# mcomunita/syncfusion

Measured on AMD Instinct MI355X. Metric: U-Net denoise steps/sec (batch x 2 s@22.05 kHz), higher is better.
Workload: dtype bf16; 1 GPU; BASELINE configs[1]: batch=8/GPU, 50-step DDIM (v-sampler) denoising of 2 s @ 22.05 kHz clips (L0=45056 = 44*1024, cropped to 44100), bf16, embedding_scale=1.0 (1 U-Net eval/step), dummy cond; this run timed 1568 consecutive sampler steps (the cost of a step does not depend on the schedule length); batch_per_gpu=8, L0=45056, hip_graph=True, weights_broadcast_bytes=0, gathered_clips=8

## Files before the change

include/syncfusion_amd.h:

```cpp
#ifndef SYNCFUSION_AMD_H
#define SYNCFUSION_AMD_H

#include <stdint.h>

#ifdef __cplusplus
extern "C" {
#endif

#define SF_MAX_DEPTH 12

enum {
  SF_OK = 0,
  SF_ERR_INVALID = 1,
  SF_ERR_MISSING_WEIGHT = 2,
  SF_ERR_SHAPE = 3,
  SF_ERR_HIP = 4,
  SF_ERR_WORKSPACE = 5,
  SF_ERR_UNSUPPORTED = 6
};

enum { SF_UP_NEAREST_CONV3 = 0, SF_UP_TRANSPOSE = 1 };
enum { SF_F32 = 0, SF_BF16 = 1, SF_F16 = 2, SF_F32X = 3 };

typedef struct {
// ... 129 lines not shown
                        int B, int L, int C, int N, int taps, int pad, float *dx, float *dw, float *db, float *dgb, void *ws,
                        int64_t ws_bytes, void *stream);
int64_t sf_op_gn_silu_train_stats_floats(int B, int L, int C, int groups);
int sf_op_gn_silu_train(const float *x, const float *gamma, const float *beta, int groups, float eps, int B, int L, int C, float *act, float *stats,
                        void *stream);
int sf_op_conv1d_bwd_cl_act(const float *x, const float *act, const float *stats , const float *w, const float *gamma, const float *beta,
                            int groups, float eps, const float *dy, int B, int L, int C, int N, int taps, int pad, float *dx, float *dw, float *db,
                            float *dgb, void *ws, int64_t ws_bytes, void *stream);
int sf_op_conv1d_bwd_cl_x(int dtype, const float *x, const float *act, const float *stats, const float *w, const float *gamma, const float *beta,
                          int groups, float eps, const float *dy, int B, int L, int C, int N, int taps, int pad, float *dx, float *dw, float *db,
                          float *dgb, void *ws, int64_t ws_bytes, void *stream);
int64_t sf_op_conv1d_dgrad_pack_bytes(int C, int N, int taps);
int sf_op_conv1d_train_fwd(int dtype, const float *x, const float *w, const float *bias, const float *gamma, const float *beta, int groups, float eps,
                           const float *residual, int B, int L, int C, int N, int taps, int pad, float *out, void *dgrad_pack, int64_t dgrad_pack_bytes,
                           void *ws, int64_t ws_bytes, void *stream);
int sf_op_conv1d_bwd_cl_p(int dtype, const float *x, const float *act, const float *stats, const float *w, const void *dgrad_pack, const float *gamma,
                          const float *beta, int groups, float eps, const float *dy, const float *dx_add, int B, int L, int C, int N, int taps, int pad,
                          float *dx, float *dw, float *db, float *dgb, void *ws, int64_t ws_bytes, void *stream);
int sf_op_conv1d_train_images(int dtype, const float *w, int B, int L, int C, int N, int taps, int pad, int groups);
int sf_op_conv1d_variant(int dtype, int B, int L, int C, int N, int taps, int stride, int pad, int upsample, int groups, char *label, int label_bytes);
int sf_op_conv1d_bwd_variant(int dtype, int B, int L, int C, int N, int taps, int pad, char *label, int label_bytes);
int sf_train_pack_many(const void *desc_dev, int n_items, int total_tiles, void *stream);
int sf_op_conv1d_train_fwd_pk(int dtype, const float *x, const float *w, const float *fw, const void *fwx, const float *bias, const float *gamma,
                              const float *beta, int groups, float eps, const float *residual, int B, int L, int C, int N, int taps, int pad, float *out,
                              void *ws, int64_t ws_bytes, void *stream);
int sf_op_ln_modulate_bwd_add(const float *x, const float *scale_shift, const float *dy, const float *dx_add, float eps, int B, int L, int C, float *dx,
                              float *dss, void *ws, int64_t ws_bytes, void *stream);
int64_t sf_op_length_sums_workspace_bytes(int B, int L, int C);
int sf_op_length_sums(const float *x, const float *y , int B, int L, int C, float *out , void *ws, int64_t ws_bytes,
                      void *stream);
int64_t sf_op_ln_modulate_bwd_workspace_bytes(int B, int L, int C);
int sf_op_ln_modulate_bwd(const float *x, const float *scale_shift, const float *dy, float eps, int B, int L, int C, float *dx, float *dss,
                          void *ws, int64_t ws_bytes, void *stream);
int sf_op_attention_bwd(const float *q, const float *kv, const float *out, const float *dout, int B, int L, int heads, int head_dim, float *dq,
                        float *dkv, void *ws, int64_t ws_bytes, void *stream);
int sf_op_attention_fwd_lse(const float *q, const float *kv, int B, int L, int heads, int head_dim, float *out, float *lse, void *stream);
int sf_op_attention_fwd_lse_x(int dtype, const float *q, const float *kv, int B, int L, int heads, int head_dim, float *out, float *lse, void *stream);
int sf_op_attention_bwd_lse(const float *q, const float *kv, const float *out, const float *dout, const float *lse, int B, int L, int heads, int head_dim,
                            float *dq, float *dkv, void *ws, int64_t ws_bytes, void *stream);
int sf_op_attention_bwd_lse_x(int dtype, const float *q, const float *kv, const float *out, const float *dout, const float *lse, int B, int L, int heads,
                              int head_dim, float *dq, float *dkv, void *ws, int64_t ws_bytes, void *stream);
int sf_bench_conv1d(int dtype, int B, int L, int C, int N, int taps, int upsample, int path, int tile, int sk, int iters,
                    float *ms_out);
int64_t sf_op_resnet_mod_cb_workspace_bytes(int B, int L, int C);
int sf_op_resnet_mod_cb(int dtype, const void *x, const float *w1, const float *b1, const float *w2, const float *b2, const float *gn1_g,
                        const float *gn1_b, const float *gn2_g, const float *gn2_b, int groups, float eps_gn, const float *scale_shift,
                        float eps_ln, int B, int L, int C, int kb , void *h_out, void *m_out,
                        void *ws, int64_t ws_bytes, void *stream);
int64_t sf_op_resnet_mod_cbd_workspace_bytes(int B, int L, int C, int C2);
int sf_op_resnet_mod_cbd(int dtype, const void *x, const float *w1, const float *b1, const float *w2, const float *b2, const float *gn1_g,
                         const float *gn1_b, const float *gn2_g, const float *gn2_b, int groups, float eps_gn, const float *scale_shift,
                         float eps_ln, int B, int L, int C, const float *w_inj, const float *b_inj, const void *ctx, int ctx_ld, int C2,
                         const float *badd, void *h_out, void *m_out, void *z_out, float *stats_out, void *ws, int64_t ws_bytes, void *stream);
int64_t sf_op_inject_prenorm_proj_workspace_bytes(int B, int L, int C, int C2, int N);
int sf_op_inject_prenorm_proj(int dtype, const void *m, const void *ctx, const float *w_inj, const float *b_inj, const float *gamma,
                              const float *beta, float eps, const float *w_q, int B, int L, int C, int C2, int N, void *z_out, void *q_out,
                              int *fused_out, void *ws, int64_t ws_bytes, void *stream);
int sf_bench_conv_cb(int dtype, int B, int L, int C, int groups, int kb, int cold, int iters, float *ms );
int sf_op_gn_silu(int dtype, const void *x, const float *gamma, const float *beta, int groups, float eps, int B, int L, int C, void *out,
                  void *ws, int64_t ws_bytes, void *stream);
int sf_op_ln_modulate(int dtype, const void *x, const float *scale_shift , float eps,
                      int B, int L, int C, void *out, void *stream);
int sf_op_attention(int dtype, const void *q, const void *kv, int B, int L, int heads, int head_dim, void *out, void *stream);


typedef struct {
  int32_t N, T, Hi, Wi;
  int32_t cin, cin_ld;
  int32_t cout, cout_ld;
  int32_t kt, kh, kw;
  int32_t sh, sw;
  int32_t pt, ph, pw;
} sf_vconv_desc;
int64_t sf_op_vconv_workspace_bytes(const sf_vconv_desc *desc );
int sf_op_vconv_fwd(const sf_vconv_desc *desc, const float *x, const float *w, float *y, void *ws, int64_t ws_bytes, void *stream);
int sf_op_vconv_bwd(const sf_vconv_desc *desc, const float *x, const float *w, const float *dy, float *dx, float *dw, void *ws, int64_t ws_bytes,
                    void *stream);
int64_t sf_op_bn_train_workspace_bytes(int64_t rows, int C);
int sf_op_bn_train_fwd(const float *x, const float *res, int64_t rows, int C, int ld, const float *gamma, const float *beta, float eps, float momentum,
                       float *running_mean, float *running_var, int64_t *num_batches_tracked, int relu, float *y, float *save_mean, float *save_invstd,
                       void *ws, int64_t ws_bytes, void *stream);
int sf_op_bn_train_bwd(const float *x, const float *y, const float *dy, int64_t rows, int C, int ld, const float *gamma, const float *save_mean,
                       const float *save_invstd, float *dx, float *dres, float *dgamma, float *dbeta, void *ws, int64_t ws_bytes, void *stream);
int64_t sf_op_bn_sync_workspace_bytes(int64_t rows, int C);
int sf_op_bn_sync_stats(const float *x, int64_t rows, int C, int ld, float *local_stats, void *ws, int64_t ws_bytes, void *stream);
int sf_op_bn_sync_fwd_apply(const float *x, const float *res, int64_t rows, int C, int ld, const float *gathered_stats, const int64_t *row_counts, int world,
                            const float *gamma, const float *beta, float eps, float momentum, float *running_mean, float *running_var,
                            int64_t *num_batches_tracked, int relu, float *y, float *save_mean, float *save_invstd, void *ws, int64_t ws_bytes,
                            void *stream);
int sf_op_bn_sync_bwd_sums(const float *x, const float *y, const float *dy, int64_t rows, int C, int ld, const float *save_mean, const float *save_invstd,
                           float *local_sums, float *dgamma, float *dbeta, void *ws, int64_t ws_bytes, void *stream);
int sf_op_bn_sync_bwd_apply(const float *x, const float *y, const float *dy, int64_t rows, int C, int ld, const float *gathered_sums,
                            const int64_t *row_counts, int world, const float *gamma, const float *save_mean, const float *save_invstd, float *dx,
                            float *dres, void *ws, int64_t ws_bytes, void *stream);
int sf_op_video_to_cl(const float *x, int N, int C, int T, int H, int W, int ld, float *out, void *stream);
int sf_op_video_pool(const float *x, int64_t NT, int HW, int C, int ld, float *out, void *stream);
int sf_op_video_pool_bwd(const float *dout, int64_t NT, int HW, int C, int ld, float *dx, void *stream);

int64_t sf_op_onset_loss_workspace_bytes(int64_t n);
int sf_op_onset_bce_fwd(const float *z, const float *t, int64_t n, float *loss, float *stats, void *ws, int64_t ws_bytes, void *stream);
int sf_op_onset_bce_bwd(const float *z, const float *t, const float *stats, const float *g, int64_t n, float *dz, void *stream);
int sf_op_onset_metrics(const float *z, const float *t, int N, int T, float threshold, double *out, void *ws, int64_t ws_bytes, void *stream);

int64_t sf_op_onset_test_workspace_bytes(int N, int T);
int sf_op_onset_test_step(const float *logits, const float *labels, int N, int T, float logit_threshold, float metric_threshold, int64_t clip0,
                          int64_t capacity, int32_t *pred_count, int32_t *pred_frames, int32_t *target_count, int32_t *target_frames,
// ... 41 lines not shown
```

syncfusion_amd/_lib.py:

```python
from __future__ import annotations

import ctypes as C
import os
from typing import Dict, Iterable, List, Optional, Sequence, Tuple

import torch

SF_MAX_DEPTH = 12
SF_F32, SF_BF16, SF_F16, SF_F32X = 0, 1, 2, 3
UPSAMPLE_MODES = {"nearest": 0, "transpose": 1}
DTYPES = {"fp32": SF_F32, "float32": SF_F32, "f32": SF_F32, "bf16": SF_BF16, "bfloat16": SF_BF16, "fp16": SF_F16, "float16": SF_F16, "f16": SF_F16, "half": SF_F16,
          "fp32x": SF_F32X}

_HERE = os.path.dirname(os.path.abspath(__file__))
LIB_PATH = os.environ.get("SF_LIB_PATH") or os.path.join(_HERE, "lib", "libsyncfusion_amd.so")


class SfTensor(C.Structure):
    _fields_ = [("name", C.c_char_p), ("data", C.c_void_p), ("numel", C.c_int64)]


class UnetConfig(C.Structure):
    _fields_ = [
        ("n_layers", C.c_int32), ("in_channels", C.c_int32),
# ... 52 lines not shown
    "sf_onsetnet_create": (_I, [C.POINTER(SfTensor), _I, _I, _P, C.POINTER(_P)]),
    "sf_onsetnet_destroy": (None, [_P]),
    "sf_onsetnet_workspace_bytes": (_L, [_P, _I, _I, _I, _I]),
    "sf_onsetnet_forward": (_I, [_P, _P, _I, _I, _I, _I, _P, _P, _L, _P]),
    "sf_onsetnet_debug_enable": (_I, [_P, _P, _L]),
    "sf_onsetnet_debug_count": (_I, [_P]),
    "sf_onsetnet_debug_detail": (_I, [_P, _I, C.POINTER(C.c_int32), _I]),
    "sf_onsetnet_debug_path": (_I, [_P, _I]),
    "sf_onsetnet_debug_info": (_I, [_P, _I, C.c_char_p, _I, C.POINTER(_L), C.POINTER(_L), C.POINTER(C.c_int32)]),
    "sf_onsets_to_track": (_I, [_P, _I, _I, _P, _F, _F, _F, _P, _I, _P]),
    "sf_frames_preprocess": (_I, [_P, _I, _I, _I, _I, _I, _I, _P, _P, _P, _P]),
    "sf_frames_augment_workspace_bytes": (_L, [_I, _I, _I, _I]),
    "sf_frames_augment": (_I, [_P, _I, _I, _I, _I, _I, _I, _I, _I, _P, _P, _P, _P, _P, _P, _L, _P]),
    "sf_times_to_track": (_I, [_P, _P, _I, C.c_double, _I, _I, _P, _P]),
    "sf_cut_prefix_crop": (_I, [_P, _P, _I, _I, _I, _I, _P, _P, _P]),
    "sf_resampler_create": (_I, [_I, _I, _I, _F, C.POINTER(_P)]),
    "sf_resampler_destroy": (None, [_P]),
    "sf_resampler_out_length": (_I, [_P, _I]),
    "sf_resampler_forward": (_I, [_P, _P, _I, _I, _P, _P]),
    "sf_op_conv1d_cl": (_I, [_I, _P, _P, _P, _P, _P, _I, _F, _P, _I, _I, _I, _I, _I, _I, _I, _I, _P, _P, _L, _P]),
    "sf_op_conv1d_bwd_workspace_bytes": (_L, [_I, _I, _I, _I, _I, _I]),
    "sf_op_conv1d_bwd_cl": (_I, [_P, _P, _P, _P, _I, _F, _P, _I, _I, _I, _I, _I, _I, _P, _P, _P, _P, _P, _L, _P]),
    "sf_op_conv1d_bwd_cl_act": (_I, [_P, _P, _P, _P, _P, _P, _I, _F, _P, _I, _I, _I, _I, _I, _I, _P, _P, _P, _P, _P, _L, _P]),
    "sf_op_conv1d_bwd_cl_x": (_I, [_I, _P, _P, _P, _P, _P, _P, _I, _F, _P, _I, _I, _I, _I, _I, _I, _P, _P, _P, _P, _P, _L, _P]),
    "sf_op_conv1d_dgrad_pack_bytes": (_L, [_I, _I, _I]),
    "sf_op_conv1d_train_fwd": (_I, [_I, _P, _P, _P, _P, _P, _I, _F, _P, _I, _I, _I, _I, _I, _I, _P, _P, _L, _P, _L, _P]),
    "sf_op_conv1d_bwd_cl_p": (_I, [_I, _P, _P, _P, _P, _P, _P, _P, _I, _F, _P, _P, _I, _I, _I, _I, _I, _I, _P, _P, _P, _P, _P, _L, _P]),
    "sf_op_conv1d_train_images": (_I, [_I, _P, _I, _I, _I, _I, _I, _I, _I]),
    "sf_op_conv1d_variant": (_I, [_I, _I, _I, _I, _I, _I, _I, _I, _I, _I, C.c_char_p, _I]),
    "sf_op_conv1d_bwd_variant": (_I, [_I, _I, _I, _I, _I, _I, _I, C.c_char_p, _I]),
    "sf_train_pack_many": (_I, [_P, _I, _I, _P]),
    "sf_op_conv1d_train_fwd_pk": (_I, [_I, _P, _P, _P, _P, _P, _P, _P, _I, _F, _P, _I, _I, _I, _I, _I, _I, _P, _P, _L, _P]),
    "sf_op_ln_modulate_bwd_add": (_I, [_P, _P, _P, _P, _F, _I, _I, _I, _P, _P, _P, _L, _P]),
    "sf_op_gn_silu_train_stats_floats": (_L, [_I, _I, _I, _I]),
    "sf_op_gn_silu_train": (_I, [_P, _P, _P, _I, _F, _I, _I, _I, _P, _P, _P]),
    "sf_op_ln_modulate_bwd_workspace_bytes": (_L, [_I, _I, _I]),
    "sf_op_ln_modulate_bwd": (_I, [_P, _P, _P, _F, _I, _I, _I, _P, _P, _P, _L, _P]),
    "sf_op_attention_bwd": (_I, [_P, _P, _P, _P, _I, _I, _I, _I, _P, _P, _P, _L, _P]),
    "sf_op_attention_fwd_lse": (_I, [_P, _P, _I, _I, _I, _I, _P, _P, _P]),
    "sf_op_attention_fwd_lse_x": (_I, [_I, _P, _P, _I, _I, _I, _I, _P, _P, _P]),
    "sf_op_attention_bwd_lse": (_I, [_P, _P, _P, _P, _P, _I, _I, _I, _I, _P, _P, _P, _L, _P]),
    "sf_op_attention_bwd_lse_x": (_I, [_I, _P, _P, _P, _P, _P, _I, _I, _I, _I, _P, _P, _P, _L, _P]),
    "sf_op_length_sums_workspace_bytes": (_L, [_I, _I, _I]),
    "sf_op_length_sums": (_I, [_P, _P, _I, _I, _I, _P, _P, _L, _P]),
    "sf_bench_conv1d": (_I, [_I, _I, _I, _I, _I, _I, _I, _I, _I, _I, _I, C.POINTER(C.c_float)]),
    "sf_op_gn_silu": (_I, [_I, _P, _P, _P, _I, _F, _I, _I, _I, _P, _P, _L, _P]),
    "sf_op_inject_prenorm_proj_workspace_bytes": (_L, [_I, _I, _I, _I, _I]),
    "sf_op_inject_prenorm_proj": (_I, [_I, _P, _P, _P, _P, _P, _P, _F, _P, _I, _I, _I, _I, _I, _P, _P, _P, _P, _L, _P]),
    "sf_op_resnet_mod_cb_workspace_bytes": (_L, [_I, _I, _I]),
    "sf_op_resnet_mod_cb": (_I, [_I, _P, _P, _P, _P, _P, _P, _P, _P, _P, _I, _F, _P, _F, _I, _I, _I, _I, _P, _P, _P, _L, _P]),
    "sf_op_resnet_mod_cbd_workspace_bytes": (_L, [_I, _I, _I, _I]),
    "sf_op_resnet_mod_cbd": (_I, [_I, _P, _P, _P, _P, _P, _P, _P, _P, _P, _I, _F, _P, _F, _I, _I, _I, _P, _P, _P, _I, _I, _P, _P, _P, _P, _P, _P,
                                  _L, _P]),
    "sf_bench_conv_cb": (_I, [_I, _I, _I, _I, _I, _I, _I, _I, C.POINTER(C.c_float)]),
    "sf_op_ln_modulate": (_I, [_I, _P, _P, _F, _I, _I, _I, _P, _P]),
    "sf_op_attention": (_I, [_I, _P, _P, _I, _I, _I, _I, _P, _P]),
    "sf_op_vconv_workspace_bytes": (_L, [C.POINTER(VConvDesc)]),
    "sf_op_vconv_fwd": (_I, [C.POINTER(VConvDesc), _P, _P, _P, _P, _L, _P]),
    "sf_op_vconv_bwd": (_I, [C.POINTER(VConvDesc), _P, _P, _P, _P, _P, _P, _L, _P]),
    "sf_op_bn_train_workspace_bytes": (_L, [_L, _I]),
    "sf_op_bn_train_fwd": (_I, [_P, _P, _L, _I, _I, _P, _P, _F, _F, _P, _P, _P, _I, _P, _P, _P, _P, _L, _P]),
    "sf_op_bn_train_bwd": (_I, [_P, _P, _P, _L, _I, _I, _P, _P, _P, _P, _P, _P, _P, _P, _L, _P]),
    "sf_op_bn_sync_workspace_bytes": (_L, [_L, _I]),
    "sf_op_bn_sync_stats": (_I, [_P, _L, _I, _I, _P, _P, _L, _P]),
    "sf_op_bn_sync_fwd_apply": (_I, [_P, _P, _L, _I, _I, _P, _P, _I, _P, _P, _F, _F, _P, _P, _P, _I, _P, _P, _P, _P, _L, _P]),
    "sf_op_bn_sync_bwd_sums": (_I, [_P, _P, _P, _L, _I, _I, _P, _P, _P, _P, _P, _P, _L, _P]),
    "sf_op_bn_sync_bwd_apply": (_I, [_P, _P, _P, _L, _I, _I, _P, _P, _I, _P, _P, _P, _P, _P, _P, _L, _P]),
    "sf_op_video_to_cl": (_I, [_P, _I, _I, _I, _I, _I, _I, _P, _P]),
    "sf_op_video_pool": (_I, [_P, _L, _I, _I, _I, _P, _P]),
    "sf_op_video_pool_bwd": (_I, [_P, _L, _I, _I, _I, _P, _P]),
    "sf_op_onset_loss_workspace_bytes": (_L, [_L]),
    "sf_op_onset_bce_fwd": (_I, [_P, _P, _L, _P, _P, _P, _L, _P]),
    "sf_op_onset_bce_bwd": (_I, [_P, _P, _P, _P, _L, _P, _P]),
    "sf_op_onset_metrics": (_I, [_P, _P, _I, _I, _F, _P, _P, _L, _P]),
    "sf_op_onset_test_workspace_bytes": (_L, [_I, _I]),
    "sf_op_onset_test_step": (_I, [_P, _P, _I, _I, _F, _F, _L, _L, _P, _P, _P, _P, _P, _P, _L, _P]),
    "sf_optim_workspace_bytes": (_L, [_I]),
    "sf_optim_adamw_step": (_I, [_P, _I, _I, _P, _I, _I, _P, _P, _L, _P]),
    "sf_audio_features_create": (_I, [_I, _I, _I, _I, _P, _P, _P, _L, C.POINTER(_P)]),
    "sf_audio_features_destroy": (None, [_P]),
    "sf_audio_features_workspace_bytes": (_L, [_P, _I, _I]),
    "sf_logmel_forward": (_I, [_P, _P, _I, _I, _F, _F, _P, _P, _P, _L, _P]),
    "sf_onset_detect": (_I, [_P, _P, _I, _I, _F, _F, _I, _I, _I, _I, _I, _I, _F, _I, _I, _P, _P, _P, _P, _P, _P, _L, _P]),
    "sf_audio_features_create_framed": (_I, [_I, _I, _I, _I, _P, _P, _P, _L, C.POINTER(_P)]),
    "sf_logmel_examples_count": (_I, [_P, _I, _I]),
    "sf_logmel_examples_forward": (_I, [_P, _P, _I, _I, _I, _F, _P, _P, _P]),
    "sf_vggish_create": (_I, [_I, _P, _I, _P, _I, _I, _I, _P, _P, _P, _P, _P, C.POINTER(_P)]),
    "sf_vggish_destroy": (None, [_P]),
    "sf_vggish_max_examples": (_I, [_P]),
    "sf_vggish_workspace_bytes": (_L, [_P, _I]),
    "sf_vggish_forward": (_I, [_P, _P, _I, _P, _P, _P, _L, _P]),
    "sf_op_maxpool2x2_cl": (_I, [_P, _L, _I, _I, _I, _P, _P]),
    "sf_op_moments": (_I, [_P, _L, _I, _P, _P, _P]),
}

_lib: Optional[C.CDLL] = None


class SyncFusionAmdError(RuntimeError):
    pass


def load() -> C.CDLL:
    global _lib
    if _lib is not None:
        return _lib
# ... 56 lines not shown
```

syncfusion_amd/csrc/capi_misc.cpp:

```cpp
#include <algorithm>
#include <cstring>
#include <cstdlib>
#include <cmath>
#include <exception>

#include "engine_common.h"

using namespace sf;

#define SF_API_BEGIN try {
#define SF_API_END                  \
  }                                 \
  catch (const EngineError &e) {    \
    return e.code;                  \
  }                                 \
  catch (const std::exception &e) { \
    set_error("%s", e.what());      \
    return SF_ERR_INVALID;          \
  }

extern "C" {

const char *sf_version(void) { return "syncfusion_amd 0.1.0 (gfx950)"; }
const char *sf_last_error(void) { return get_error(); }
// ... 580 lines not shown
  Workspace wk(ws, ws_bytes);
  const int64_t es = 2;
  char *wp = static_cast<char *>(wk.alloc(2 * (int64_t)C * C * 3 * es));
  void *wp1 = wp, *wp2 = wp + (int64_t)C * C * 3 * es;
  void *act = wk.alloc(M * C * es);
  void *h = h_out ? h_out : wk.alloc(M * C * es);
  void *m = m_out ? m_out : wk.alloc(M * C * es);
  float *stats = stats_out ? stats_out : static_cast<float *>(wk.alloc((int64_t)B * 32 * 64 * 2 * 4));
  if (w_inj) {
    void *wi = wk.alloc((int64_t)C * (C + C2) * es);
    ai.w = wi;
    ai.src = ai.res = m;
    if (!conv_gemm_supported(dtype, ai)) fail(SF_ERR_UNSUPPORTED, "InjectChannels shape outside the GEMM kernels' coverage");
    SF_HIP(launch_pack_rows(dtype, w_inj, C, C + C2, C + C2, nullptr, wi, C + C2, s));
  }
  SF_HIP(launch_pack_conv_cb(dtype, w1, C, C, wp1, s));
  SF_HIP(launch_pack_conv_cb(dtype, w2, C, C, wp2, s));
  SF_HIP(launch_gn_silu(dtype, x, C, B, L, C, groups, gn1_g, gn1_b, eps_gn, act, C, s));
  ConvCbArgs a;
  a.src = act;
  a.src_ld = C;
  a.wp = wp1;
  a.B = B;
  a.L = L;
  a.C = a.N = C;
  a.G = groups;
  const CbGnPlan gp = cb_gn_plan(L);
  a.nch = gp.nch;
  a.chunk_rows = gp.chunk_rows;
  a.epi = 1;
  a.out = h;
  a.out_ld = C;
  a.bias = b1;
  a.stats_out = stats;
  SF_HIP(launch_conv_cb(dtype, a, s));
  a.src = h;
  a.wp = wp2;
  a.pro = 1;
  a.stats = stats;
  a.gamma = gn2_g;
  a.beta = gn2_b;
  a.eps = eps_gn;
  a.epi = 2;
  a.out = m;
  a.bias = b2;
  a.stats_out = nullptr;
  a.res = x;
  a.res_ld = C;
  a.ss = scale_shift;
  a.ss_ld = 2 * C;
  a.eps_ln = eps_ln;
  SF_HIP(launch_conv_cb(dtype, a, s));
  if (w_inj) SF_HIP(launch_conv_gemm(dtype, ai, s));
  return SF_OK;
  SF_API_END
}

int64_t sf_op_inject_prenorm_proj_workspace_bytes(int B, int L, int C, int C2, int N) {
  if (B < 1 || L < 1 || C < 32 || C2 < 0 || N < 8) return -1;
  const int64_t M = (int64_t)B * L, K1 = C + (C2 + 31) / 32 * 32;
  return (int64_t)C * K1 * 2 + (int64_t)N * C * 2 + M * C * 2 + M * (C / 32) * 8 + (int64_t)(2 * N + C) * 4 + 4096;
}

int sf_op_inject_prenorm_proj(int dtype, const void *m, const void *ctx, const float *w_inj, const float *b_inj, const float *gamma,
                              const float *beta, float eps, const float *w_q, int B, int L, int C, int C2, int N, void *z_out, void *q_out,
                              int *fused_out, void *ws, int64_t ws_bytes, void *stream) {
  SF_API_BEGIN
  if (!m || !w_inj || !b_inj || !gamma || !beta || !w_q || !z_out || !q_out || !ws) fail(SF_ERR_INVALID, "null argument");
  if (dtype != BF16 && dtype != F16) fail(SF_ERR_UNSUPPORTED, "16-bit dtypes only");
  if (C % 32 || C2 % 32 || N % 32 || (C2 > 0 && !ctx)) fail(SF_ERR_UNSUPPORTED, "C, C2 and N must be multiples of 32");
  const int64_t need = sf_op_inject_prenorm_proj_workspace_bytes(B, L, C, C2, N);
  if (need < 0 || ws_bytes < need) fail(SF_ERR_WORKSPACE, "workspace too small: need %lld bytes", (long long)need);
  hipStream_t s = static_cast<hipStream_t>(stream);
  Workspace wk(ws, ws_bytes);
  const int64_t M = (int64_t)B * L;
  const int K1 = C + C2;
  void *w1 = wk.alloc((int64_t)C * K1 * 2), *w2 = wk.alloc((int64_t)N * C * 2), *tmp = wk.alloc(M * C * 2);
  float *rowpart = static_cast<float *>(wk.alloc(M * (C / 32) * 8));
  float *bias2 = static_cast<float *>(wk.alloc((int64_t)N * 4)), *colsum = static_cast<float *>(wk.alloc((int64_t)N * 4));
  SF_HIP(launch_pack_rows(dtype, w_inj, C, K1, K1, nullptr, w1, K1, s));
  SF_HIP(launch_pack_rows(dtype, w_q, N, C, C, gamma, w2, C, s));
  SF_HIP(launch_fold_bias(w_q, N, C, beta, nullptr, bias2, s));
  SF_HIP(launch_row_sums(dtype, w2, N, C, colsum, s));
  ConvGemmArgs a;
  a.src = m;
  a.src_ld = C;
  a.src2 = ctx;
  a.src2_ld = C2;
  a.w = w1;
  a.bias = b_inj;
  a.M = (int)M;
  a.N = a.n_store = C;
  a.K = K1;
  a.cin = C;
  a.cin2 = C2;
  a.taps = 1;
  a.Lout = a.Lsrc = L;
  a.out = z_out;
  a.out_ld = C;
  a.res = m;
  a.res_ld = C;
  ConvGemmArgs q;
  q.src = z_out;
  q.src_ld = C;
  q.w = w2;
  q.bias = bias2;
// ... 119 lines not shown
```

syncfusion_amd/csrc/conv_thin.hip:

```cpp
#include <cstdlib>
#include <type_traits>

#include "common.h"
#include "kernels.h"

namespace sf {
namespace {

static int thin_max_waves(int C) {
  static const int v32 = [] {
    const char *e = tune_env("SF_THIN_WAVES32");
    const int w = e ? atoi(e) : 8;
    return w >= 16 ? 16 : (w >= 8 ? 8 : 4);
  }();
  static const int v64 = [] {
    const char *e = tune_env("SF_THIN_WAVES64");
    const int w = e ? atoi(e) : 8;
    return w >= 16 ? 16 : (w >= 8 ? 8 : 4);
  }();
  return C == 32 ? v32 : (C == 64 ? v64 : 16);
}

constexpr int kThinMaxTiles = 64;
constexpr int kThinMaxG = 16;
// ... 86 lines not shown
  __device__ __forceinline__ static K8x zero() {
    K8x r;
    const u32x4 z = {0u, 0u, 0u, 0u};
    r.h = __builtin_bit_cast(f16x8, z);
    r.l = r.h;
    return r;
  }
};
__device__ __forceinline__ void mma_step_x3(f32x16 &accM, f32x16 &accL, const K8x &a, const K8x &b) { x3_mfma<X3_F16>(a.h, a.l, b.h, b.l, accM, accL); }
__device__ __forceinline__ void x3_fold(f32x16 &accM, const f32x16 &accL) {
#pragma unroll
  for (int i = 0; i < 16; ++i) accM[i] = fmaf(accL[i], X3P<X3_F16>::INV, accM[i]);
}

template <int CTRL, int ROW_MASK> __device__ __forceinline__ float dpp_mov(float v) {
  return __int_as_float(__builtin_amdgcn_update_dpp(0, __float_as_int(v), CTRL, ROW_MASK, 0xf, false));
}
__device__ __forceinline__ float2 half_sums(float v) {
  v += dpp_mov<0xb1, 0xf>(v);
  v += dpp_mov<0x4e, 0xf>(v);
  v += dpp_mov<0x124, 0xf>(v);
  v += dpp_mov<0x128, 0xf>(v);
  v += dpp_mov<0x142, 0xa>(v);
  return make_float2(__int_as_float(__builtin_amdgcn_readlane(__float_as_int(v), 31)),
                     __int_as_float(__builtin_amdgcn_readlane(__float_as_int(v), 63)));
}
__device__ __forceinline__ float half_sum32(float v, int half) {
  v += dpp_mov<0xb1, 0xf>(v);
  v += dpp_mov<0x4e, 0xf>(v);
  v += dpp_mov<0x124, 0xf>(v);
  v += dpp_mov<0x128, 0xf>(v);
  v += dpp_mov<0x142, 0xa>(v);
  const float lo = __int_as_float(__builtin_amdgcn_readlane(__float_as_int(v), 31));
  const float hi = __int_as_float(__builtin_amdgcn_readlane(__float_as_int(v), 63));
  return half ? hi : lo;
}

template <bool FAST = false>
__device__ __forceinline__ float2 gn_merge_n(const float *__restrict__ sl, int G, int nch, int chunk_rows, int L, int cpg, float eps,
                                             int lane32) {
  float n = 0.f, mean = 0.f, m2 = 0.f;
  for (int i = lane32; i < nch; i += 32) {
    const int rows = min(chunk_rows, L - i * chunk_rows);
    welford_merge_t<FAST>(n, mean, m2, (float)rows * (float)cpg, sl[(size_t)i * G * 2], sl[(size_t)i * G * 2 + 1]);
  }
#pragma unroll
  for (int off = 16; off > 0; off >>= 1) {
    const float nb = __shfl_down(n, off, 32), mb = __shfl_down(mean, off, 32), qb = __shfl_down(m2, off, 32);
    welford_merge_t<FAST>(n, mean, m2, nb, mb, qb);
  }
  const float mu = __shfl(mean, 0, 32), var = div_t<FAST>(__shfl(m2, 0, 32), __shfl(n, 0, 32));
  return make_float2(mu, rsqrtf(var + eps));
}

template <typename T> struct K4;
template <> struct K4<bf16> {
  uint2 raw;
  __device__ __forceinline__ float get(int i) const {
    const unsigned int w = i < 2 ? raw.x : raw.y;
    return __uint_as_float((i & 1) ? (w & 0xffff0000u) : (w << 16));
  }
  __device__ __forceinline__ static K4 load(const bf16 *p) {
    K4 r;
    r.raw = *reinterpret_cast<const uint2 *>(p);
    return r;
  }
  __device__ __forceinline__ static K4 zero() {
    K4 r;
    r.raw = make_uint2(0u, 0u);
    return r;
  }
};
template <> struct K4<f16> {
  typedef __attribute__((ext_vector_type(4))) _Float16 f16x4;
  f16x4 v;
  __device__ __forceinline__ float get(int i) const { return (float)v[i]; }
  __device__ __forceinline__ static K4 load(const f16 *p) {
    K4 r;
    r.v = *reinterpret_cast<const f16x4 *>(p);
    return r;
  }
  __device__ __forceinline__ static K4 zero() {
    K4 r;
    r.v = f16x4{(f16)0.f, (f16)0.f, (f16)0.f, (f16)0.f};
    return r;
  }
};
template <> struct K4<float> {
  f32x4 v;
  __device__ __forceinline__ float get(int i) const { return v[i]; }
  __device__ __forceinline__ static K4 load(const float *p) {
    K4 r;
    r.v = *reinterpret_cast<const f32x4 *>(p);
    return r;
  }
  __device__ __forceinline__ static K4 zero() {
    K4 r;
    r.v = f32x4{0.f, 0.f, 0.f, 0.f};
    return r;
  }
};

template <typename T, int CIN, int TAPS, int C2, int PRO, int NOUT, bool X3 = false>
__global__ __launch_bounds__(X3 ? 512 : 1024) void conv_thin_kernel(const ConvThinArgs a) {
  static_assert(!X3 || sizeof(T) == 4, "split mode: fp32 activations");
  constexpr int E = 8;
// ... 344 lines not shown
  nw = (nw / NCB) * NCB;
  if (((a.rw >> a.up_shift) + 3) * (CIN / 8) > 6 * nw * 64) return hipErrorInvalidValue;
  hipLaunchKernelGGL(kern, dim3(a.B * a.nchw), dim3(nw * 64), lds, s, a);
  return hipGetLastError();
}

struct ThinShape {
  int cin, taps, c2, pro, nout;
};
constexpr ThinShape kThinShapes[] = {
    {8, 3, 0, 1, 8},   {32, 3, 0, 1, 32},  {64, 3, 0, 1, 64},
    {8, 1, 8, 2, 8},   {32, 1, 32, 2, 32}, {64, 1, 32, 2, 64}, {64, 1, 64, 2, 64},
    {32, 1, 0, 0, 32}, {64, 1, 0, 0, 64},  {128, 1, 0, 0, 64},
    {32, 3, 0, 0, 8},  {64, 3, 0, 0, 32},  {64, 3, 0, 0, 64},
};

static hipError_t thin_dispatch_x3(const ConvThinArgs &a, hipStream_t s) {
#define SF_THINX(CC, TT, C22, PP, NN) \
  if (a.C == CC && a.taps == TT && a.C2 == C22 && a.pro == PP && a.N == NN) return thin_go<float, CC, TT, C22, PP, NN, true>(a, s)
  SF_THINX(32, 3, 0, 1, 32);
  SF_THINX(64, 3, 0, 1, 64);
  SF_THINX(32, 1, 32, 2, 32);
  SF_THINX(64, 1, 32, 2, 64);
  SF_THINX(64, 1, 64, 2, 64);
  SF_THINX(32, 1, 0, 0, 32);
  SF_THINX(64, 1, 0, 0, 64);
  SF_THINX(128, 1, 0, 0, 64);
  SF_THINX(64, 3, 0, 0, 32);
  SF_THINX(64, 3, 0, 0, 64);
#undef SF_THINX
  return hipErrorInvalidValue;
}

template <typename T> hipError_t thin_dispatch(const ConvThinArgs &a, hipStream_t s) {
#define SF_THIN(CC, TT, C22, PP, NN) \
  if (a.C == CC && a.taps == TT && a.C2 == C22 && a.pro == PP && a.N == NN) return thin_go<T, CC, TT, C22, PP, NN>(a, s)
  SF_THIN(8, 3, 0, 1, 8);
  SF_THIN(32, 3, 0, 1, 32);
  SF_THIN(64, 3, 0, 1, 64);
  SF_THIN(8, 1, 8, 2, 8);
  SF_THIN(32, 1, 32, 2, 32);
  SF_THIN(64, 1, 32, 2, 64);
  SF_THIN(64, 1, 64, 2, 64);
  SF_THIN(32, 1, 0, 0, 32);
  SF_THIN(64, 1, 0, 0, 64);
  SF_THIN(128, 1, 0, 0, 64);
  SF_THIN(32, 3, 0, 0, 8);
  SF_THIN(64, 3, 0, 0, 32);
  SF_THIN(64, 3, 0, 0, 64);
#undef SF_THIN
  return hipErrorInvalidValue;
}

template <typename T, int C, int C2, bool X3 = false>
__global__ __launch_bounds__(X3 ? 512 : 1024) void thin_tail_kernel(const ThinTailArgs a) {
  static_assert(!X3 || sizeof(T) == 4, "split mode: fp32 activations");
  constexpr int E = 8;
  constexpr int QC = C / E;
  constexpr int S2 = 3 * QC, NST2 = (S2 + 1) / 2;
  constexpr int NSTM = (C + 15) / 16;
  constexpr int SC = C2 / E, NSTC = (SC + 1) / 2;
  constexpr int NCB = (C + 31) / 32;
  constexpr int K2 = 3 * C, K3 = C + C2;
  constexpr int P2 = K2 + E, P3 = K3 + E;
  constexpr int SROW = C + E;
  constexpr int NV = 6;
  constexpr bool FAST = !std::is_same<T, float>::value;

  extern __shared__ __align__(16) unsigned char smem[];
  float *sc = reinterpret_cast<float *>(smem);
  float *sh = sc + C;
  float *lsc = sh + C;
  float *lsh = lsc + C;
  float *ep = lsh + C;
  float *part = ep + 128;
  T *w2s = reinterpret_cast<T *>(part + kThinMaxTiles * kThinMaxG * 2);
  T *w3s = w2s + C * P2;
  T *tile = w3s + C * P3;
  f16 *w2H = reinterpret_cast<f16 *>(w2s), *w2L = w2H + C * P2;
  f16 *w3H = reinterpret_cast<f16 *>(w3s), *w3L = w3H + C * P3;
  f16 *tileH = reinterpret_cast<f16 *>(tile), *tileL = tileH + (size_t)(a.rw + 4) * SROW;

  const int tid = threadIdx.x, lane = tid & 63, wave = tid >> 6, NW = blockDim.x >> 6;
  const int half = lane >> 5, l32 = lane & 31;
  const int b = blockIdx.x / a.nchw, ch = blockIdx.x - b * a.nchw;
  const int r0 = ch * a.rw;
  const int rows = min(a.rw, a.L - r0);
  const int ntile = (rows + 31) >> 5;
  const int cpg = C / a.G;
  const T *src = static_cast<const T *>(a.h);

  const int total = (rows + 2) * QC;
  K8<T> xin[NV];
#pragma unroll
  for (int i = 0; i < NV; ++i) {
    const int idx = tid + i * blockDim.x;
    const int rr = idx / QC, q = idx - rr * QC;
    const int pos = r0 - 1 + rr;
    const bool ok = idx < total && pos >= 0 && pos < a.L;
    xin[i] = ok ? K8<T>::load(src + ((size_t)b * a.L + pos) * C + q * E) : K8<T>::zero();
  }
  for (int i = tid; i < C * (K2 / E); i += blockDim.x) {
    const int r = i / (K2 / E), v = i - r * (K2 / E);
    const K8<T> w = K8<T>::load(static_cast<const T *>(a.w2) + (size_t)r * K2 + v * E);
    if constexpr (X3) K8x::from(w).store(w2H + r * P2 + v * E, w2L + r * P2 + v * E);
    else w.store(w2s + r * P2 + v * E);
  }
  for (int i = tid; i < C * (K3 / E); i += blockDim.x) {
    const int r = i / (K3 / E), v = i - r * (K3 / E);
    const K8<T> w = K8<T>::load(static_cast<const T *>(a.w3) + (size_t)r * K3 + v * E);
    if constexpr (X3) K8x::from(w).store(w3H + r * P3 + v * E, w3L + r * P3 + v * E);
    else w.store(w3s + r * P3 + v * E);
  }
  for (int g = tid >> 5; g < a.G; g += blockDim.x >> 5) {
    const float2 st = gn_merge_n<FAST>(a.stats_in + ((size_t)b * a.nch_in * a.G + g) * 2, a.G, a.nch_in, a.chunk_in, a.L, cpg, a.eps_gn, l32);
    if (l32 < cpg) {
      const int c = g * cpg + l32;
      const float s = st.y * a.gamma[c];
      sc[c] = s;
      sh[c] = a.beta[c] - st.x * s;
    }
  }
  if (tid < C) {
    lsc[tid] = 1.0f + a.ss[(size_t)b * a.ss_ld + tid];
    lsh[tid] = a.ss[(size_t)b * a.ss_ld + C + tid];
    ep[tid] = a.bias2[tid];
    ep[64 + tid] = a.bias3[tid] + (a.badd ? a.badd[(size_t)b * a.badd_ld + tid] : 0.f);
  }
  __syncthreads();
#pragma unroll
  for (int i = 0; i < NV; ++i) {
    const int idx = tid + i * blockDim.x;
    if (idx < total) {
      const int rr = idx / QC, q = idx - rr * QC;
      const int pos = r0 - 1 + rr;
      const bool ok = pos >= 0 && pos < a.L;
      K8<T> v = xin[i];
#pragma unroll
      for (int e = 0; e < E; ++e) {
        const float y = fmaf(v.get(e), sc[q * E + e], sh[q * E + e]);
        v.set(e, ok ? silu_t<FAST>(y) : 0.f);
      }
      if constexpr (X3) K8x::from(v).store(tileH + rr * SROW + q * E, tileL + rr * SROW + q * E);
      else v.store(tile + rr * SROW + q * E);
    }
  }
  __syncthreads();

  for (int t = wave; t < ntile; t += NW) {
    const int row_l = t * 32 + l32;
    const bool rvalid = row_l < rows;
    const size_t grow = (size_t)b * a.L + r0 + (rvalid ? row_l : 0);
    K8<T> cf[NSTC > 0 ? NSTC : 1];
#pragma unroll
    for (int i = 0; i < NSTC; ++i) {
      const int q2 = 2 * i + half;
      cf[i] = (rvalid && q2 < SC) ? K8<T>::load(static_cast<const T *>(a.ctx) + grow * a.ctx_ld + q2 * E) : K8<T>::zero();
    }
    K4<T> rxf[NCB][4];
#pragma unroll
    for (int cb = 0; cb < NCB; ++cb)
#pragma unroll
      for (int v = 0; v < 4; ++v) {
        const int c0 = cb * 32 + half * 4 + 8 * v;
        rxf[cb][v] = (c0 < C && rvalid) ? K4<T>::load(static_cast<const T *>(a.x) + grow * C + c0) : K4<T>::zero();
      }
    f32x16 acc[NCB];
#pragma unroll
    for (int cb = 0; cb < NCB; ++cb)
#pragma unroll
      for (int i = 0; i < 16; ++i) acc[cb][i] = 0.f;
    const int prow = rvalid ? row_l : 0;
    if constexpr (X3) {
      f32x16 accL[NCB];
#pragma unroll
      for (int cb = 0; cb < NCB; ++cb)
#pragma unroll
        for (int i = 0; i < 16; ++i) accL[cb][i] = 0.f;
#pragma unroll
      for (int s = 0; s < NST2; ++s) {
// ... 196 lines not shown
            pp[1] = q;
          }
        }
      } else {
        const float cnt = (float)vrows * (float)cpg;
#pragma unroll
        for (int cb = 0; cb < NCB; ++cb)
#pragma unroll
          for (int v = 0; v < 4; ++v) {
            const float2 hs = half_sums((xs[cb][v][0] + xs[cb][v][1]) + (xs[cb][v][2] + xs[cb][v][3]));
            const float m = div_t<FAST>(cpg == 8 ? hs.x + hs.y : (half ? hs.y : hs.x), cnt);
            float q = 0.f;
#pragma unroll
            for (int e = 0; e < 4; ++e) {
              const float d = rvalid ? xs[cb][v][e] - m : 0.f;
              q = fmaf(d, d, q);
            }
            const float2 hq = half_sums(q);
            const float qq = cpg == 8 ? hq.x + hq.y : (half ? hq.y : hq.x);
            if (l32 == 0 && (cpg == 4 || half == 0)) {
              float *pp = part + ((size_t)t * a.G + (cb * 32 + half * 4 + 8 * v) / cpg) * 2;
              pp[0] = m;
              pp[1] = qq;
            }
          }
      }
    }
  }
  if (a.stats_out) {
    __syncthreads();
    for (int g = wave; g < a.G; g += NW) {
      const bool on = lane < ntile;
      const float *pp = part + ((size_t)(on ? lane : 0) * a.G + g) * 2;
      const float n_t = on ? (float)min(32, rows - lane * 32) * (float)cpg : 0.f;
      const float m_t = on ? pp[0] : 0.f, q_t = on ? pp[1] : 0.f;
      const float2 sn = half_sums(n_t), sm = half_sums(n_t * m_t);
      const float n = sn.x + sn.y, mean = div_t<FAST>(sm.x + sm.y, n);
      const float d = m_t - mean;
      const float2 sq2 = half_sums(fmaf(n_t * d, d, q_t));
      if (lane == 0) {
        float *so = a.stats_out + (((size_t)b * a.nchw + ch) * a.G + g) * 2;
        so[0] = mean;
        so[1] = sq2.x + sq2.y;
      }
    }
  }
}

template <typename T> size_t tail_lds_bytes(int C, int C2, int rw) {
  return (size_t)(4 * C + 128 + kThinMaxTiles * kThinMaxG * 2) * sizeof(float) +
         ((size_t)C * (3 * C + 8) + (size_t)C * (C + C2 + 8) + (size_t)(rw + 4) * (C + 8)) * sizeof(T);
}

template <typename T, int C, int C2, bool X3 = false> hipError_t tail_go(const ThinTailArgs &a, hipStream_t s) {
  const size_t lds = tail_lds_bytes<T>(C, C2, a.rw);
  auto kern = thin_tail_kernel<T, C, C2, X3>;
  if (lds > 64 * 1024) {
    static bool raised = false;
    if (!raised) {
      hipError_t e = hipFuncSetAttribute(reinterpret_cast<const void *>(kern), hipFuncAttributeMaxDynamicSharedMemorySize, 160 * 1024);
      if (e != hipSuccess) return e;
      raised = true;
    }
  }
  int nw = (a.rw + 31) / 32;
  if (nw > thin_max_waves(C)) nw = thin_max_waves(C);
  if (X3 && nw > 8) nw = 8;
  if ((a.rw + 2) * (C / 8) > 6 * nw * 64) return hipErrorInvalidValue;
  hipLaunchKernelGGL(kern, dim3(a.B * a.nchw), dim3(nw * 64), lds, s, a);
  return hipGetLastError();
}

template <typename T> hipError_t tail_dispatch(const ThinTailArgs &a, hipStream_t s) {
  if (a.C == 8 && a.C2 == 8) return tail_go<T, 8, 8>(a, s);
  if (a.C == 32 && a.C2 == 32) return tail_go<T, 32, 32>(a, s);
  if (a.C == 64 && a.C2 == 32) return tail_go<T, 64, 32>(a, s);
  if (a.C == 64 && a.C2 == 64) return tail_go<T, 64, 64>(a, s);
  return hipErrorInvalidValue;
}

}

bool thin_tail_supported(int dt, const ThinTailArgs &a) {
  const bool shape = (a.C == 8 && a.C2 == 8) || (a.C == 32 && a.C2 == 32) || (a.C == 64 && (a.C2 == 32 || a.C2 == 64));
  if (!shape || a.rw < 32 || a.rw % 32 || a.rw > 32 * kThinMaxTiles) return false;
  if (a.G < 1 || a.G > kThinMaxG || a.C % a.G) return false;
  const int cpg = a.C / a.G;
  if (a.C == 8 ? cpg != 1 : (cpg != 4 && cpg != 8)) return false;
  if (!a.ss || !a.stats_in) return false;
  {
    int nw = (a.rw + 31) / 32;
    if (nw > thin_max_waves(a.C)) nw = thin_max_waves(a.C);
    if ((a.rw + 2) * (a.C / 8) > 6 * nw * 64) return false;
  }
  const size_t lds = dt == F32 ? tail_lds_bytes<float>(a.C, a.C2, a.rw) : tail_lds_bytes<bf16>(a.C, a.C2, a.rw);
  return lds <= 160 * 1024;
}

hipError_t launch_thin_tail(int dt, const ThinTailArgs &a, hipStream_t s) {
  if (!thin_tail_supported(dt, a)) return hipErrorInvalidValue;
  if (d0_tail_supported(a)) return launch_d0_tail(dt, a, s);
  if (dt == F32 && a.x3) {
    if (a.C == 32 && a.C2 == 32) return tail_go<float, 32, 32, true>(a, s);
    if (a.C == 64 && a.C2 == 32) return tail_go<float, 64, 32, true>(a, s);
    if (a.C == 64 && a.C2 == 64) return tail_go<float, 64, 64, true>(a, s);
  }
  return SF_DISPATCH_T(dt, tail_dispatch<T>(a, s));
}

ThinPlan conv_thin_plan(int B, int L, int C) {
  ThinPlan p;
  static const int rows8 = [] {
    const char *e = tune_env("SF_THIN_ROWS8");
    const int v = e ? atoi(e) : 0;
    return v > 0 ? v : 0;
  }();
  static const int rows_cap = [] {
    const char *e = tune_env("SF_THIN_MAXROWS");
    const int v = e ? atoi(e) : 0;
    return v > 0 ? v : 352;
  }();
  static const int rows32 = [] {
    const char *e = tune_env("SF_THIN_MAXROWS32");
    const int v = e ? atoi(e) : 0;
    return v > 0 ? v : 512;
  }();
  const int max_rows = C <= 8 ? (rows8 > 0 ? rows8 : (d0_enabled(B, L) ? 992 : 2048)) : (C == 32 && rows32 > 0 ? rows32 : rows_cap);
  static const int wgs = [] {
    const char *e = tune_env("SF_THIN_WGS");
    const int v = e ? atoi(e) : 0;
    return v > 0 ? v : 256;
  }();
  long target = ((long)B * L + wgs - 1) / wgs;
  int rw = (int)((target + 31) / 32) * 32;
  if (rw < 32) rw = 32;
  if (rw > max_rows) rw = max_rows;
  p.rw = rw;
  p.nchw = (L + rw - 1) / rw;
  return p;
}

bool conv_thin_supported(int dt, const ConvThinArgs &a) {
  bool shape = false;
  for (const ThinShape &t : kThinShapes) shape = shape || (a.C == t.cin && a.taps == t.taps && a.C2 == t.c2 && a.pro == t.pro && a.N == t.nout);
  if (!shape) return false;
// ... 31 lines not shown
```

Baseline: 540.4 steps/s.

## Stage thin-tail weights and GroupNorm stats up front with overlapped loads

Adds an AHEAD variant of the thin-level tail kernel for 16-bit dtypes with C>=32 and small row windows. It issues the weight loads into registers in batches, and folds the GroupNorm statistics (with an FMA/reciprocal Welford merge) while those loads are in flight. The goal is to hide global-load latency during the prologue. It also enforces a minimum wave count, tunable by env, for these small blocks, and exposes a standalone C API entry point for the tail. The cost is more register pressure and a lower launch bound of 512.

Result: faster. 549.9 steps/s (median of 6 runs) (+1.8%).

```diff
diff --git a/include/syncfusion_amd.h b/include/syncfusion_amd.h
--- a/include/syncfusion_amd.h
+++ b/include/syncfusion_amd.h
@@ -205,6 +205,11 @@
                          const float *gn1_b, const float *gn2_g, const float *gn2_b, int groups, float eps_gn, const float *scale_shift,
                          float eps_ln, int B, int L, int C, const float *w_inj, const float *b_inj, const void *ctx, int ctx_ld, int C2,
                          const float *badd, void *h_out, void *m_out, void *z_out, float *stats_out, void *ws, int64_t ws_bytes, void *stream);
+int64_t sf_op_thin_tail_workspace_bytes(int dtype, int C, int C2);
+int sf_op_thin_tail(int dtype, const void *h, const void *x, const void *ctx, int ctx_ld, int c2_real, int C2, const float *stats_in, int nch_in,
+                    int chunk_in, const float *w2, const float *b2, const float *gn_g, const float *gn_b, int groups, float eps_gn,
+                    const float *scale_shift, float eps_ln, const float *w_inj, const float *b_inj, const float *badd, int B, int L, int C, int rw,
+                    void *z_out, float *stats_out, int *rw_out, void *ws, int64_t ws_bytes, void *stream);
 int64_t sf_op_inject_prenorm_proj_workspace_bytes(int B, int L, int C, int C2, int N);
 int sf_op_inject_prenorm_proj(int dtype, const void *m, const void *ctx, const float *w_inj, const float *b_inj, const float *gamma,
                               const float *beta, float eps, const float *w_q, int B, int L, int C, int C2, int N, void *z_out, void *q_out,
diff --git a/syncfusion_amd/_lib.py b/syncfusion_amd/_lib.py
--- a/syncfusion_amd/_lib.py
+++ b/syncfusion_amd/_lib.py
@@ -128,6 +128,9 @@
     "sf_op_resnet_mod_cbd_workspace_bytes": (_L, [_I, _I, _I, _I]),
     "sf_op_resnet_mod_cbd": (_I, [_I, _P, _P, _P, _P, _P, _P, _P, _P, _P, _I, _F, _P, _F, _I, _I, _I, _P, _P, _P, _I, _I, _P, _P, _P, _P, _P, _P,
                                   _L, _P]),
+    "sf_op_thin_tail_workspace_bytes": (_L, [_I, _I, _I]),
+    "sf_op_thin_tail": (_I, [_I, _P, _P, _P, _I, _I, _I, _P, _I, _I, _P, _P, _P, _P, _I, _F, _P, _F, _P, _P, _P, _I, _I, _I, _I, _P, _P,
+                             C.POINTER(C.c_int), _P, _L, _P]),
     "sf_bench_conv_cb": (_I, [_I, _I, _I, _I, _I, _I, _I, _I, C.POINTER(C.c_float)]),
     "sf_op_ln_modulate": (_I, [_I, _P, _P, _F, _I, _I, _I, _P, _P]),
     "sf_op_attention": (_I, [_I, _P, _P, _I, _I, _I, _I, _P, _P]),
diff --git a/syncfusion_amd/csrc/capi_misc.cpp b/syncfusion_amd/csrc/capi_misc.cpp
--- a/syncfusion_amd/csrc/capi_misc.cpp
+++ b/syncfusion_amd/csrc/capi_misc.cpp
@@ -656,6 +656,72 @@
   a.eps_ln = eps_ln;
   SF_HIP(launch_conv_cb(dtype, a, s));
   if (w_inj) SF_HIP(launch_conv_gemm(dtype, ai, s));
+  return SF_OK;
+  SF_API_END
+}
+
+int64_t sf_op_thin_tail_workspace_bytes(int dtype, int C, int C2) {
+  if ((dtype != F32 && dtype != BF16 && dtype != F16) || C < 1 || C2 < 0) return -1;
+  Workspace dry(nullptr, 0);
+  dry.alloc((int64_t)C * 3 * C * (int64_t)dsize(dtype));
+  dry.alloc((int64_t)C * (C + C2) * (int64_t)dsize(dtype));
+  return dry.used();
+}
+
+int sf_op_thin_tail(int dtype, const void *h, const void *x, const void *ctx, int ctx_ld, int c2_real, int C2, const float *stats_in, int nch_in,
+                    int chunk_in, const float *w2, const float *b2, const float *gn_g, const float *gn_b, int groups, float eps_gn,
+                    const float *scale_shift, float eps_ln, const float *w_inj, const float *b_inj, const float *badd, int B, int L, int C, int rw,
+                    void *z_out, float *stats_out, int *rw_out, void *ws, int64_t ws_bytes, void *stream) {
+  SF_API_BEGIN
+  if (!h || !x || !stats_in || !w2 || !b2 || !gn_g || !gn_b || !scale_shift || !w_inj || !b_inj || !z_out || !ws) fail(SF_ERR_INVALID, "null argument");
+  if (dtype != F32 && dtype != BF16 && dtype != F16) fail(SF_ERR_UNSUPPORTED, "dtype: fp32, bf16 or fp16");
+  if (B < 1 || L < 1 || C < 8) fail(SF_ERR_INVALID, "bad shape");
+  if (C2 < 0 || C2 % 8 || c2_real < 0 || c2_real > C2 || (C2 > 0 && (!ctx || ctx_ld < C2 || ctx_ld % 8))) fail(SF_ERR_INVALID, "context operands inconsistent");
+  if (nch_in < 1 || chunk_in < 1 || (int64_t)(nch_in - 1) * chunk_in >= L || (int64_t)nch_in * chunk_in < L)
+    fail(SF_ERR_INVALID, "nch_in chunks of chunk_in rows do not tile L = %d", L);
+  if (rw < 0 || rw % 32) fail(SF_ERR_UNSUPPORTED, "rw must be a multiple of 32 (0: the plan's choice)");
+  ThinTailArgs t;
+  if (rw == 0) rw = conv_thin_plan(B, L, C).rw;
+  t.rw = rw;
+  t.nchw = (L + rw - 1) / rw;
+  t.h = h;
+  t.x = x;
+  t.ctx = ctx;
+  t.ctx_ld = ctx_ld;
+  t.bias2 = b2;
+  t.bias3 = b_inj;
+  t.gamma = gn_g;
+  t.beta = gn_b;
+  t.stats_in = stats_in;
+  t.ss = scale_shift;
+  t.ss_ld = 2 * C;
+  t.badd = badd;
+  t.badd_ld = C;
+  t.out = z_out;
+  t.stats_out = stats_out;
+  t.B = B;
+  t.L = L;
+  t.C = C;
+  t.C2 = C2;
+  t.G = groups;
+  t.nch_in = nch_in;
+  t.chunk_in = chunk_in;
+  t.eps_gn = eps_gn;
+  t.eps_ln = eps_ln;
+  if (groups < 1 || !thin_tail_supported(dtype, t)) fail(SF_ERR_UNSUPPORTED, "shape outside the thin-level tail's coverage (C / C2 = 8/8, 32/32, 64/32, 64/64; 4 or 8 channels per group)");
+  const int64_t need = sf_op_thin_tail_workspace_bytes(dtype, C, C2);
+  if (need < 0 || ws_bytes < need) fail(SF_ERR_WORKSPACE, "workspace too small: need %lld bytes", (long long)need);
+  hipStream_t s = static_cast<hipStream_t>(stream);
+  Workspace wk(ws, ws_bytes);
+  const int64_t es = (int64_t)dsize(dtype);
+  void *wp2 = wk.alloc((int64_t)C * 3 * C * es), *wp3 = wk.alloc((int64_t)C * (C + C2) * es);
+  t.w2 = wp2;
+  t.w3 = wp3;
+  SF_HIP(launch_pack_conv(dtype, w2, C, C, 0, C, 3, C, nullptr, wp2, 3 * C, 0, s));
+  SF_HIP(launch_pack_conv(dtype, w_inj, C, C + c2_real, 0, C, 1, C, nullptr, wp3, C + C2, 0, s));
+  if (C2) SF_HIP(launch_pack_conv(dtype, w_inj, C, C + c2_real, C, c2_real, 1, C2, nullptr, wp3, C + C2, C, s));
+  SF_HIP(launch_thin_tail(dtype, t, s));
+  if (rw_out) *rw_out = rw;
   return SF_OK;
   SF_API_END
 }
diff --git a/syncfusion_amd/csrc/conv_thin.hip b/syncfusion_amd/csrc/conv_thin.hip
--- a/syncfusion_amd/csrc/conv_thin.hip
+++ b/syncfusion_amd/csrc/conv_thin.hip
@@ -162,6 +162,69 @@
   const float mu = __shfl(mean, 0, 32), var = div_t<FAST>(__shfl(m2, 0, 32), __shfl(n, 0, 32));
   return make_float2(mu, rsqrtf(var + eps));
 }
+
+__device__ __forceinline__ void welford_merge_fma(float &n, float &mean, float &m2, float nb, float mb, float m2b) {
+  if (nb <= 0.f) return;
+  const float tot = n + nb, r = __builtin_amdgcn_rcpf(tot);
+  const float delta = mb - mean;
+  mean = fmaf(nb * r, delta, mean);
+  m2 += fmaf(n * nb * r, delta * delta, m2b);
+  n = tot;
+}
+template <int NG, int NP> struct GnAhead {
+  float m[NG][NP], q[NG][NP], gam[NG], bet[NG];
+};
+template <int NG, int NP>
+__device__ __forceinline__ void gn_ahead_load(GnAhead<NG, NP> &p, const float *__restrict__ sb ,
+                                              const float *__restrict__ gamma, const float *__restrict__ beta, int G, int nch, int cpg, int g0,
+                                              int hw, int nhw, int lane32) {
+#pragma unroll
+  for (int gi = 0; gi < NG; ++gi) {
+    const int g = min(g0 + hw + gi * nhw, G - 1);
+#pragma unroll
+    for (int k = 0; k < NP; ++k) {
+      const int i = min(lane32 + 32 * k, nch - 1);
+      p.m[gi][k] = sb[((size_t)i * G + g) * 2];
+      p.q[gi][k] = sb[((size_t)i * G + g) * 2 + 1];
+    }
+    const int c = g * cpg + min(lane32, cpg - 1);
+    p.gam[gi] = gamma[c];
+    p.bet[gi] = beta[c];
+  }
+}
+template <bool FAST, int NG, int NP>
+__device__ __forceinline__ void gn_ahead_fold(const GnAhead<NG, NP> &p, const float *__restrict__ sb, int G, int nch, int chunk_rows, int L,
+                                              int cpg, float eps, int g0, int hw, int nhw, int lane32, float *sc, float *sh) {
+  static_assert(FAST, "16-bit kernels: the reciprocal form of the merge");
+#pragma unroll
+  for (int gi = 0; gi < NG; ++gi) {
+    const int g = g0 + hw + gi * nhw;
+    if (g >= G) break;
+    float n = 0.f, mean = 0.f, m2 = 0.f;
+#pragma unroll
+    for (int k = 0; k < NP; ++k) {
+      const int i = lane32 + 32 * k;
+      if (i < nch) welford_merge_fma(n, mean, m2, (float)min(chunk_rows, L - i * chunk_rows) * (float)cpg, p.m[gi][k], p.q[gi][k]);
+    }
+    for (int i = lane32 + 32 * NP; i < nch; i += 32) {
+      const int rows = min(chunk_rows, L - i * chunk_rows);
+      welford_merge_fma(n, mean, m2, (float)rows * (float)cpg, sb[((size_t)i * G + g) * 2], sb[((size_t)i * G + g) * 2 + 1]);
+    }
+#pragma unroll
+    for (int off = 16; off > 0; off >>= 1) {
+      const float nb = __shfl_down(n, off, 32), mb = __shfl_down(mean, off, 32), qb = __shfl_down(m2, off, 32);
+      welford_merge_fma(n, mean, m2, nb, mb, qb);
+    }
+    const float mu = __shfl(mean, 0, 32), var = div_t<FAST>(__shfl(m2, 0, 32), __shfl(n, 0, 32));
+    if (lane32 < cpg) {
+      const int c = g * cpg + lane32;
+      const float s = rsqrtf(var + eps) * p.gam[gi];
+      sc[c] = s;
+      sh[c] = p.bet[gi] - mu * s;
+    }
+  }
+}
+constexpr int kGnAheadG = 2, kGnAheadP = 2;
 
 template <typename T> struct K4;
 template <> struct K4<bf16> {
@@ -612,9 +675,13 @@
   return hipErrorInvalidValue;
 }
 
-template <typename T, int C, int C2, bool X3 = false>
-__global__ __launch_bounds__(X3 ? 512 : 1024) void thin_tail_kernel(const ThinTailArgs a) {
+template <typename T, int C> constexpr bool tail_ahead() { return sizeof(T) == 2 && C >= 32; }
+template <int C> constexpr int tail_wb() { return C >= 64 ? 10 : 4; }
+
+template <typename T, int C, int C2, bool X3 = false, bool AHEAD = false>
+__global__ __launch_bounds__((X3 || AHEAD) ? 512 : 1024) void thin_tail_kernel(const ThinTailArgs a) {
   static_assert(!X3 || sizeof(T) == 4, "split mode: fp32 activations");
+  static_assert(!AHEAD || tail_ahead<T, C>(), "up-front staging: the 16-bit MFMA levels");
   constexpr int E = 8;
   constexpr int QC = C / E;
   constexpr int S2 = 3 * QC, NST2 = (S2 + 1) / 2;
@@ -660,6 +727,66 @@
     const bool ok = idx < total && pos >= 0 && pos < a.L;
     xin[i] = ok ? K8<T>::load(src + ((size_t)b * a.L + pos) * C + q * E) : K8<T>::zero();
   }
+  if constexpr (AHEAD) {
+    const int tc = min(tid, C - 1);
+    const float m_sc = a.ss[(size_t)b * a.ss_ld + tc], m_sh = a.ss[(size_t)b * a.ss_ld + C + tc];
+    const float m_b2 = a.bias2[tc], m_b3 = a.bias3[tc], m_ba = a.badd ? a.badd[(size_t)b * a.badd_ld + tc] : 0.f;
+    const float *sb = a.stats_in + (size_t)b * a.nch_in * a.G * 2;
+    const int hw = tid >> 5, nhw = blockDim.x >> 5;
+    GnAhead<kGnAheadG, kGnAheadP> gp;
+    gn_ahead_load(gp, sb, a.gamma, a.beta, a.G, a.nch_in, cpg, 0, hw, nhw, l32);
+    constexpr int W2V = C * (K2 / E), WV = W2V + C * (K3 / E);
+    const T *w2g = static_cast<const T *>(a.w2), *w3g = static_cast<const T *>(a.w3);
+    auto wsrc = [&](int i) -> const T * {
+      if (i < W2V) {
+        const int r = i / (K2 / E), v = i - r * (K2 / E);
+        return w2g + (size_t)r * K2 + v * E;
+      }
+      const int i3 = i - W2V, r = i3 / (K3 / E), v = i3 - r * (K3 / E);
+      return w3g + (size_t)r * K3 + v * E;
+    };
+    auto wdst = [&](int i) -> T * {
+      if (i < W2V) {
+        const int r = i / (K2 / E), v = i - r * (K2 / E);
+        return w2s + r * P2 + v * E;
+      }
+      const int i3 = i - W2V, r = i3 / (K3 / E), v = i3 - r * (K3 / E);
+      return w3s + r * P3 + v * E;
+    };
+    constexpr int WB = tail_wb<C>();
+    K8<T> wq[WB];
+    auto w_issue = [&](int base) {
+#pragma unroll
+      for (int j = 0; j < WB; ++j) {
+        const int first = base + j * (int)blockDim.x;
+        wq[j] = first < WV ? K8<T>::load(wsrc(min(first + tid, WV - 1))) : K8<T>::zero();
+      }
+    };
+    auto w_store = [&](int base) {
+#pragma unroll
+      for (int j = 0; j < WB; ++j) {
+        const int i = base + j * (int)blockDim.x + tid;
+        if (i < WV) wq[j].store(wdst(i));
+      }
+    };
+    w_issue(0);
+    gn_ahead_fold<FAST>(gp, sb, a.G, a.nch_in, a.chunk_in, a.L, cpg, a.eps_gn, 0, hw, nhw, l32, sc, sh);
+    if (tid < C) {
+      lsc[tid] = 1.0f + m_sc;
+      lsh[tid] = m_sh;
+      ep[tid] = m_b2;
+      ep[64 + tid] = m_b3 + m_ba;
+    }
+    w_store(0);
+    for (int base = WB * (int)blockDim.x; base < WV; base += WB * (int)blockDim.x) {
+      w_issue(base);
+      w_store(base);
+    }
+    for (int g0 = kGnAheadG * nhw; g0 < a.G; g0 += kGnAheadG * nhw) {
+      gn_ahead_load(gp, sb, a.gamma, a.beta, a.G, a.nch_in, cpg, g0, hw, nhw, l32);
+      gn_ahead_fold<FAST>(gp, sb, a.G, a.nch_in, a.chunk_in, a.L, cpg, a.eps_gn, g0, hw, nhw, l32, sc, sh);
+    }
+  } else {
   for (int i = tid; i < C * (K2 / E); i += blockDim.x) {
     const int r = i / (K2 / E), v = i - r * (K2 / E);
     const K8<T> w = K8<T>::load(static_cast<const T *>(a.w2) + (size_t)r * K2 + v * E);
@@ -686,6 +813,7 @@
     lsh[tid] = a.ss[(size_t)b * a.ss_ld + C + tid];
     ep[tid] = a.bias2[tid];
     ep[64 + tid] = a.bias3[tid] + (a.badd ? a.badd[(size_t)b * a.badd_ld + tid] : 0.f);
+  }
   }
   __syncthreads();
 #pragma unroll
@@ -988,9 +1116,24 @@
          ((size_t)C * (3 * C + 8) + (size_t)C * (C + C2 + 8) + (size_t)(rw + 4) * (C + 8)) * sizeof(T);
 }
 
-template <typename T, int C, int C2, bool X3 = false> hipError_t tail_go(const ThinTailArgs &a, hipStream_t s) {
+static bool tail_small(int C, int rw) { return (rw + 31) / 32 <= (C >= 64 ? 4 : 6); }
+
+static int tail_waves(bool ahead, bool x3, int C, int rw) {
+  static const int floor_w = [] {
+    const char *e = tune_env("SF_THIN_TAIL_MINWAVES");
+    const int w = e ? atoi(e) : 4;
+    return w < 1 ? 1 : (w > 8 ? 8 : w);
+  }();
+  int nw = (rw + 31) / 32;
+  if (nw > thin_max_waves(C)) nw = thin_max_waves(C);
+  if ((ahead || x3) && nw > 8) nw = 8;
+  if (ahead && nw < floor_w) nw = floor_w;
+  return nw;
+}
+
+template <typename T, int C, int C2, bool X3, bool AHEAD> hipError_t tail_launch(const ThinTailArgs &a, hipStream_t s) {
   const size_t lds = tail_lds_bytes<T>(C, C2, a.rw);
-  auto kern = thin_tail_kernel<T, C, C2, X3>;
+  auto kern = thin_tail_kernel<T, C, C2, X3, AHEAD>;
   if (lds > 64 * 1024) {
     static bool raised = false;
     if (!raised) {
@@ -999,12 +1142,17 @@
       raised = true;
     }
   }
-  int nw = (a.rw + 31) / 32;
-  if (nw > thin_max_waves(C)) nw = thin_max_waves(C);
-  if (X3 && nw > 8) nw = 8;
+  const int nw = tail_waves(AHEAD, X3, C, a.rw);
   if ((a.rw + 2) * (C / 8) > 6 * nw * 64) return hipErrorInvalidValue;
   hipLaunchKernelGGL(kern, dim3(a.B * a.nchw), dim3(nw * 64), lds, s, a);
   return hipGetLastError();
+}
+
+template <typename T, int C, int C2, bool X3 = false> hipError_t tail_go(const ThinTailArgs &a, hipStream_t s) {
+  if constexpr (tail_ahead<T, C>()) {
+    if (tail_small(C, a.rw)) return tail_launch<T, C, C2, X3, true>(a, s);
+  }
+  return tail_launch<T, C, C2, X3, false>(a, s);
 }
 
 template <typename T> hipError_t tail_dispatch(const ThinTailArgs &a, hipStream_t s) {
@@ -1025,8 +1173,7 @@
   if (a.C == 8 ? cpg != 1 : (cpg != 4 && cpg != 8)) return false;
   if (!a.ss || !a.stats_in) return false;
   {
-    int nw = (a.rw + 31) / 32;
-    if (nw > thin_max_waves(a.C)) nw = thin_max_waves(a.C);
+    const int nw = tail_waves(dt != F32 && a.C >= 32 && tail_small(a.C, a.rw), dt == F32 && a.x3, a.C, a.rw);
     if ((a.rw + 2) * (a.C / 8) > 6 * nw * 64) return false;
   }
   const size_t lds = dt == F32 ? tail_lds_bytes<float>(a.C, a.C2, a.rw) : tail_lds_bytes<bf16>(a.C, a.C2, a.rw);
```
